# TaceoLabs/co-snarks

Measured on NVIDIA H100. Metric: co-Groth16 proofs/sec (BN254, 2^20 constraints); MSM Mscalar/s, higher is better.
Workload: dtype u32x8 (256-bit Montgomery, integer)

## Files before the change

co_snarks_b200/csrc/cs_msm.cuh:

```cuda
#pragma once
#include <stdlib.h>
#include "cs_common.cuh"
#include "cs_curve.cuh"

namespace cs {

constexpr unsigned MSM_SLICE_MAX = 64;
constexpr unsigned MSM_ORDER_BLOCK = 256;
constexpr unsigned MSM_RED_SEG = 4;
constexpr unsigned MSM_SIGN = 0x80000000u;

template <class FrP, class Fn>
CS_D void msm_recode(const uint32_t* __restrict__ scalars, uint32_t sstride, uint32_t i, int mont, uint32_t c,
                     uint32_t W, Fn&& f) {
  Fp<FrP> s;
  const uint4* src = reinterpret_cast<const uint4*>(scalars) + (size_t)i * sstride * (FrP::N / 4);
  CS_UNROLL
  for (int k = 0; k < FrP::N / 4; k++) {
    uint4 v = src[k];
    s.l[4 * k] = v.x; s.l[4 * k + 1] = v.y; s.l[4 * k + 2] = v.z; s.l[4 * k + 3] = v.w;
  }
  if (mont) s = s.from_mont();
  const uint32_t half = 1u << (c - 1);
  const uint32_t mask = (1u << c) - 1;
  uint32_t carry = 0;
  for (uint32_t w = 0; w < W; w++) {
    uint32_t pos = w * c;
    uint32_t li = pos >> 5, sh = pos & 31;
    uint32_t lo = li < FrP::N ? s.l[li] : 0;
    uint32_t hi = li + 1 < FrP::N ? s.l[li + 1] : 0;
    uint32_t d = (__funnelshift_r(lo, hi, sh) & mask) + carry;
    uint32_t out;
    if (d > half) {
      out = ((1u << c) - d) | MSM_SIGN;
      carry = 1;
    } else {
      out = d;
      carry = 0;
    }
    f(w, out);
  }
}

CS_D bool msm_base_inf(const uint32_t* __restrict__ infmask, uint32_t k) {
  return infmask && ((infmask[k >> 5] >> (k & 31)) & 1);
}

constexpr unsigned MSM_BIN_T = 1024;
constexpr unsigned MSM_BIN_TILE = 4096;
constexpr unsigned MSM_BIN_SPAN = 1u << 15;
constexpr unsigned MSM_SCATTER_SPAN = 1u << 13;

template <class FrP>
CS_GLOBAL void __launch_bounds__(MSM_BIN_T) k_msm_bin_count(const uint32_t* __restrict__ scalars, uint32_t sstride,
                                                            uint32_t n, int mont, uint32_t c, uint32_t W,
                                                            const uint32_t* __restrict__ infmask, uint32_t offset,
                                                            uint32_t tile, uint32_t B, uint32_t* __restrict__ tab) {
  CS_DYN_SMEM(uint32_t, h);
  const uint32_t lo = blockIdx.y * MSM_BIN_SPAN + 1;
  const uint32_t span = B + 1 - lo < MSM_BIN_SPAN ? B + 1 - lo : MSM_BIN_SPAN;
  for (uint32_t k = threadIdx.x; k < span; k += blockDim.x) h[k] = 0;
  __syncthreads();
  const uint32_t i1 = (blockIdx.x + 1) * tile < n ? (blockIdx.x + 1) * tile : n;
  for (uint32_t i = blockIdx.x * tile + threadIdx.x; i < i1; i += blockDim.x) {
    if (msm_base_inf(infmask, offset + i)) continue;
    msm_recode<FrP>(scalars, sstride, i, mont, c, W, [&](uint32_t, uint32_t d) {
      const uint32_t k = (d & ~MSM_SIGN) - lo;
      if (k < span) atomicAdd(&h[k], 1u);
    });
  }
  __syncthreads();
  uint32_t* row = tab + (size_t)blockIdx.x * B + (lo - 1);
  for (uint32_t k = threadIdx.x; k < span; k += blockDim.x) row[k] = h[k];
}

constexpr unsigned MSM_BIN_SCAN_U = 16;
static CS_GLOBAL void k_msm_bin_scan(uint32_t* __restrict__ tab, uint32_t nblk, uint32_t B, uint32_t* __restrict__ count) {
  const uint32_t b = blockIdx.x * blockDim.x + threadIdx.x;
  if (b == 0) count[0] = 0;
  if (b >= B) return;
  uint32_t* col = tab + b;
  uint32_t run = 0, r = 0;
  for (; r + MSM_BIN_SCAN_U <= nblk; r += MSM_BIN_SCAN_U) {
    uint32_t v[MSM_BIN_SCAN_U];
    CS_UNROLL
    for (uint32_t u = 0; u < MSM_BIN_SCAN_U; u++) v[u] = col[(size_t)(r + u) * B];
    CS_UNROLL
    for (uint32_t u = 0; u < MSM_BIN_SCAN_U; u++) {
      col[(size_t)(r + u) * B] = run;
      run += v[u];
    }
  }
  for (; r < nblk; r++) {
    const uint32_t v = col[(size_t)r * B];
    col[(size_t)r * B] = run;
    run += v;
  }
  count[b + 1] = run;
}

template <class FrP>
CS_GLOBAL void __launch_bounds__(MSM_BIN_T) k_msm_bin_scatter(const uint32_t* __restrict__ scalars, uint32_t sstride,
                                                              uint32_t n, int mont, uint32_t c, uint32_t W,
                                                              const uint32_t* __restrict__ infmask, uint32_t offset,
                                                              uint32_t tile, uint32_t B, uint32_t nbases,
                                                              const uint32_t* __restrict__ tab,
                                                              const uint32_t* __restrict__ start,
                                                              uint32_t* __restrict__ sorted) {
  CS_DYN_SMEM(uint32_t, cur);
  const uint32_t lo = blockIdx.y * MSM_SCATTER_SPAN + 1;
  const uint32_t span = B + 1 - lo < MSM_SCATTER_SPAN ? B + 1 - lo : MSM_SCATTER_SPAN;
  const uint32_t* row = tab + (size_t)blockIdx.x * B + (lo - 1);
  for (uint32_t k = threadIdx.x; k < span; k += blockDim.x) cur[k] = start[lo + k] + row[k];
  __syncthreads();
  const uint32_t i1 = (blockIdx.x + 1) * tile < n ? (blockIdx.x + 1) * tile : n;
  for (uint32_t i = blockIdx.x * tile + threadIdx.x; i < i1; i += blockDim.x) {
    if (msm_base_inf(infmask, offset + i)) continue;
    msm_recode<FrP>(scalars, sstride, i, mont, c, W, [&](uint32_t w, uint32_t d) {
      const uint32_t k = (d & ~MSM_SIGN) - lo;
      if (k < span) sorted[atomicAdd(&cur[k], 1u)] = (w * nbases + offset + i) | (d & MSM_SIGN);
    });
  }
}

template <class F>
CS_GLOBAL void k_msm_infmask(const Affine<F>* __restrict__ table, uint32_t n, uint32_t* __restrict__ mask) {
  uint32_t wd = blockIdx.x * blockDim.x + threadIdx.x;
  if (wd * 32 >= n) return;
  uint32_t m = 0;
  for (uint32_t k = 0; k < 32 && wd * 32 + k < n; k++)
    if (table[wd * 32 + k].is_inf()) m |= 1u << k;
  mask[wd] = m;
}

constexpr unsigned MSM_SCAN_T = 1024;
constexpr unsigned MSM_SCAN_MAX_BLOCKS = 1024;
CS_D void msm_scan_terms(const uint32_t* __restrict__ count, uint32_t k, uint32_t nb1, uint32_t S, uint32_t* v) {
  uint32_t cnt = (k && k < nb1) ? count[k] : 0;
  uint32_t n0 = (cnt + S - 1) / S;
  uint32_t n1 = (n0 + S - 1) / S;
  v[0] = cnt; v[1] = n0; v[2] = n1; v[3] = (n1 + S - 1) / S;
}
static CS_GLOBAL void k_msm_scan1(const uint32_t* __restrict__ count, uint32_t nb1 , uint32_t S,
                                  uint32_t* __restrict__ start, uint32_t* __restrict__ sstart0,
                                  uint32_t* __restrict__ sstart1, uint32_t* __restrict__ sstart2, uint32_t* __restrict__ aux) {
  __shared__ uint32_t sm[4][32];
  const uint32_t t = threadIdx.x, lane = t & 31, wid = t >> 5, nwarp = blockDim.x >> 5;
  const uint32_t k = blockIdx.x * blockDim.x + t;
  uint32_t v[4], inc[4];
  msm_scan_terms(count, k, nb1, S, v);
  CS_UNROLL
  for (int q = 0; q < 4; q++) {
    uint32_t x = v[q];
    CS_UNROLL
    for (uint32_t d = 1; d < 32; d <<= 1) {
      uint32_t y = __shfl_up_sync(0xffffffffu, x, d);
      if (lane >= d) x += y;
    }
    inc[q] = x;
    if (lane == 31) sm[q][wid] = x;
  }
  __syncthreads();
  uint32_t w[4], x[4];
  CS_UNROLL
  for (int q = 0; q < 4; q++) {
    w[q] = (wid == 0 && lane < nwarp) ? sm[q][lane] : 0;
    x[q] = w[q];
    CS_UNROLL
    for (uint32_t d = 1; d < 32; d <<= 1) {
      uint32_t y = __shfl_up_sync(0xffffffffu, x[q], d);
      if (lane >= d) x[q] += y;
    }
  }
  __syncthreads();
  if (wid == 0 && lane < nwarp) {
    CS_UNROLL
    for (int q = 0; q < 4; q++) sm[q][lane] = x[q] - w[q];
    if (lane == nwarp - 1) {
      CS_UNROLL
      for (int q = 0; q < 4; q++) aux[blockIdx.x * 4 + q] = x[q];
    }
  }
  __syncthreads();
  if (k < nb1) {
    start[k] = sm[0][wid] + inc[0] - v[0];
    sstart0[k] = sm[1][wid] + inc[1] - v[1];
    sstart1[k] = sm[2][wid] + inc[2] - v[2];
    sstart2[k] = sm[3][wid] + inc[3] - v[3];
  }
}
static CS_GLOBAL void k_msm_scan2(const uint32_t* __restrict__ count, uint32_t nb1, uint32_t S,
                                  uint32_t* __restrict__ start, uint32_t* __restrict__ sstart0,
                                  uint32_t* __restrict__ sstart1, uint32_t* __restrict__ sstart2,
                                  const uint32_t* __restrict__ aux) {
  const uint32_t k = blockIdx.x * blockDim.x + threadIdx.x;
  if (k >= nb1) return;
  uint32_t off[4] = {0, 0, 0, 0};
  for (uint32_t b = 0; b < blockIdx.x; b++) {
    CS_UNROLL
    for (int q = 0; q < 4; q++) off[q] += aux[b * 4 + q];
  }
  uint32_t a = start[k] + off[0], b0 = sstart0[k] + off[1], b1 = sstart1[k] + off[2], b2 = sstart2[k] + off[3];
  start[k] = a; sstart0[k] = b0; sstart1[k] = b1; sstart2[k] = b2;
  if (k == nb1 - 1) {
    uint32_t v[4];
    msm_scan_terms(count, k, nb1, S, v);
    start[nb1] = a + v[0]; sstart0[nb1] = b0 + v[1]; sstart1[nb1] = b1 + v[2]; sstart2[nb1] = b2 + v[3];
  }
}

constexpr unsigned MSM_VIEW_T = 256;
constexpr unsigned MSM_VIEW_WORDS = MSM_VIEW_T / 32;

CS_D uint32_t popc32(uint32_t x) {
#if defined(CS_EMU)
  return (uint32_t)__builtin_popcount(x);
#else
  return __popc(x);
#endif
}
CS_D uint32_t warp_bits(bool pred) {
#if defined(CS_EMU)
  uint32_t x = pred ? 1u << (threadIdx.x & 31) : 0u;
  for (uint32_t d = 16; d > 0; d >>= 1) x += __shfl_xor_sync(0xffffffffu, x, d);
  return x;
#else
  return __ballot_sync(0xffffffffu, pred);
#endif
}

static CS_GLOBAL void k_msm_view_flags(const uint32_t* __restrict__ sorted, const uint32_t* __restrict__ src_start,
                                       uint32_t nb1, uint32_t n, const uint32_t* __restrict__ infmask, uint32_t offset,
                                       uint32_t* __restrict__ keep, uint32_t* __restrict__ blk_cnt) {
  __shared__ uint32_t cnt[MSM_VIEW_WORDS];
  const uint32_t t = threadIdx.x;
  const uint32_t p = blockIdx.x * MSM_VIEW_T + t;
  bool k = false;
  if (p < src_start[nb1]) {
    const uint32_t i = (sorted[p] & ~MSM_SIGN) % n;
    k = !((infmask[(offset + i) >> 5] >> ((offset + i) & 31)) & 1);
  }
  const uint32_t bits = warp_bits(k);
  if ((t & 31) == 0) {
    keep[(size_t)blockIdx.x * MSM_VIEW_WORDS + (t >> 5)] = bits;
    cnt[t >> 5] = popc32(bits);
  }
  __syncthreads();
  if (t == 0) {
    uint32_t c = 0;
    for (uint32_t w = 0; w < MSM_VIEW_WORDS; w++) c += cnt[w];
    blk_cnt[blockIdx.x] = c;
  }
}

static CS_GLOBAL void k_msm_view_scan(const uint32_t* __restrict__ blk_cnt, uint32_t nblk, uint32_t* __restrict__ blk_off) {
  __shared__ uint32_t sm[MSM_SCAN_T];
  const uint32_t t = threadIdx.x, T = blockDim.x;
  const uint32_t per = (nblk + T - 1) / T;
  const uint32_t lo = t * per < nblk ? t * per : nblk, hi = lo + per < nblk ? lo + per : nblk;
  uint32_t s = 0;
  for (uint32_t b = lo; b < hi; b++) s += blk_cnt[b];
  sm[t] = s;
  __syncthreads();
  for (uint32_t d = 1; d < T; d <<= 1) {
    const uint32_t v = t >= d ? sm[t - d] : 0;
    __syncthreads();
    sm[t] += v;
    __syncthreads();
  }
  uint32_t run = sm[t] - s;
  for (uint32_t b = lo; b < hi; b++) {
    const uint32_t c = blk_cnt[b];
    blk_off[b] = run;
    run += c;
  }
  if (t == T - 1) blk_off[nblk] = run;
}

CS_D uint32_t view_kept_before(uint32_t p, const uint32_t* __restrict__ keep, const uint32_t* __restrict__ blk_off) {
  const uint32_t blk = p / MSM_VIEW_T;
  uint32_t r = blk_off[blk];
  for (uint32_t w = blk * MSM_VIEW_WORDS; w < (p >> 5); w++) r += popc32(keep[w]);
  if (p & 31) r += popc32(keep[p >> 5] & ((1u << (p & 31)) - 1));
  return r;
}

static CS_GLOBAL void k_msm_view_counts(const uint32_t* __restrict__ src_start, uint32_t nb1, const uint32_t* __restrict__ keep,
                                        const uint32_t* __restrict__ blk_off, uint32_t* __restrict__ count) {
  const uint32_t b = blockIdx.x * blockDim.x + threadIdx.x;
  if (b >= nb1) return;
  count[b] = b ? view_kept_before(src_start[b + 1], keep, blk_off) - view_kept_before(src_start[b], keep, blk_off) : 0;
}

static CS_GLOBAL void k_msm_view_scatter(const uint32_t* __restrict__ sorted, uint32_t n, uint32_t nbases, uint32_t offset,
                                         const uint32_t* __restrict__ keep, const uint32_t* __restrict__ blk_off,
                                         uint32_t* __restrict__ out) {
  const uint32_t t = threadIdx.x;
  const uint32_t* kb = keep + (size_t)blockIdx.x * MSM_VIEW_WORDS;
  const uint32_t word = kb[t >> 5];
  if (!((word >> (t & 31)) & 1)) return;
  uint32_t pos = blk_off[blockIdx.x] + popc32(word & ((1u << (t & 31)) - 1));
  for (uint32_t k = 0; k < (t >> 5); k++) pos += popc32(kb[k]);
  const uint32_t e = sorted[blockIdx.x * MSM_VIEW_T + t];
  const uint32_t v = e & ~MSM_SIGN, w = v / n, i = v - w * n;
  out[pos] = (w * nbases + offset + i) | (e & MSM_SIGN);
}

CS_D uint32_t find_bucket(const uint32_t* __restrict__ arr, uint32_t nb1, uint32_t s) {
  uint32_t lo = 0, hi = nb1;
  while (hi - lo > 1) {
    uint32_t mid = (lo + hi) >> 1;
    if (arr[mid] <= s) lo = mid; else hi = mid;
  }
  return lo;
}

static CS_GLOBAL void k_msm_slice_hist(const uint32_t* __restrict__ count, const uint32_t* __restrict__ sstart0,
                                       uint32_t nb1, uint32_t S, uint32_t* __restrict__ slice_len,
                                       uint32_t* __restrict__ slice_bkt, uint32_t* __restrict__ block_hist) {
  __shared__ uint32_t h[MSM_SLICE_MAX + 1];
  for (uint32_t k = threadIdx.x; k <= MSM_SLICE_MAX; k += blockDim.x) h[k] = 0;
  __syncthreads();
  uint32_t s = blockIdx.x * blockDim.x + threadIdx.x;
  if (s < sstart0[nb1]) {
    uint32_t lo = 0, hi = nb1;
    while (hi - lo > 1) {
      uint32_t mid = (lo + hi) >> 1;
      if (sstart0[mid] <= s) lo = mid; else hi = mid;
    }
    uint32_t j = s - sstart0[lo];
    uint32_t len = count[lo] - j * S;
    if (len > S) len = S;
    slice_len[s] = len;
    slice_bkt[s] = lo;
    atomicAdd(&h[len], 1u);
  }
  __syncthreads();
  for (uint32_t k = threadIdx.x; k <= MSM_SLICE_MAX; k += blockDim.x)
    block_hist[(size_t)blockIdx.x * (MSM_SLICE_MAX + 1) + k] = h[k];
}

constexpr unsigned MSM_OFF_CHUNKS = 64;
static CS_GLOBAL void k_msm_slice_off1(const uint32_t* __restrict__ block_hist, uint32_t nblocks,
                                       uint32_t* __restrict__ chunk_sum) {
  uint32_t id = blockIdx.x * blockDim.x + threadIdx.x;
  if (id >= (MSM_SLICE_MAX + 1) * MSM_OFF_CHUNKS) return;
  uint32_t L = id / MSM_OFF_CHUNKS, ch = id % MSM_OFF_CHUNKS;
  uint32_t per = (nblocks + MSM_OFF_CHUNKS - 1) / MSM_OFF_CHUNKS;
  uint32_t lo = ch * per, hi = lo + per < nblocks ? lo + per : nblocks;
  uint32_t sum = 0;
  for (uint32_t b = lo; b < hi; b++) sum += block_hist[(size_t)b * (MSM_SLICE_MAX + 1) + L];
  chunk_sum[id] = sum;
}
static CS_GLOBAL void k_msm_slice_off2(uint32_t* __restrict__ chunk_sum, uint32_t* __restrict__ len_base) {
  uint32_t L = blockIdx.x * blockDim.x + threadIdx.x;
  if (L > MSM_SLICE_MAX) return;
  uint32_t run = 0;
  for (uint32_t c = 0; c < MSM_OFF_CHUNKS; c++) {
    uint32_t v = chunk_sum[L * MSM_OFF_CHUNKS + c];
    chunk_sum[L * MSM_OFF_CHUNKS + c] = run;
    run += v;
  }
  len_base[MSM_SLICE_MAX + 1 + L] = run;
}
static CS_GLOBAL void k_msm_slice_off3(uint32_t* __restrict__ block_hist, uint32_t nblocks,
                                       const uint32_t* __restrict__ chunk_sum, uint32_t* __restrict__ len_base) {
  uint32_t id = blockIdx.x * blockDim.x + threadIdx.x;
  if (id == 0) {
    uint32_t run = 0;
    for (int k = MSM_SLICE_MAX; k >= 0; k--) { len_base[k] = run; run += len_base[MSM_SLICE_MAX + 1 + k]; }
  }
  if (id >= (MSM_SLICE_MAX + 1) * MSM_OFF_CHUNKS) return;
  uint32_t L = id / MSM_OFF_CHUNKS, ch = id % MSM_OFF_CHUNKS;
  uint32_t per = (nblocks + MSM_OFF_CHUNKS - 1) / MSM_OFF_CHUNKS;
  uint32_t lo = ch * per, hi = lo + per < nblocks ? lo + per : nblocks;
  uint32_t run = chunk_sum[id];
  for (uint32_t b = lo; b < hi; b++) {
    uint32_t v = block_hist[(size_t)b * (MSM_SLICE_MAX + 1) + L];
    block_hist[(size_t)b * (MSM_SLICE_MAX + 1) + L] = run;
    run += v;
  }
}

static CS_GLOBAL void k_msm_slice_order(const uint32_t* __restrict__ slice_len, const uint32_t* __restrict__ slice_bkt,
                                        uint32_t nslices_max, const uint32_t* __restrict__ sstart0, uint32_t nb1,
                                        const uint32_t* __restrict__ block_off, const uint32_t* __restrict__ len_base,
                                        uint32_t* __restrict__ order, uint32_t* __restrict__ order_b) {
  __shared__ uint32_t h[MSM_SLICE_MAX + 1];
  for (uint32_t k = threadIdx.x; k <= MSM_SLICE_MAX; k += blockDim.x) h[k] = 0;
  __syncthreads();
  uint32_t s = blockIdx.x * blockDim.x + threadIdx.x;
  if (s < sstart0[nb1]) {
    uint32_t len = slice_len[s];
    uint32_t rank = atomicAdd(&h[len], 1u);
    uint32_t pos = len_base[len] + block_off[(size_t)blockIdx.x * (MSM_SLICE_MAX + 1) + len] + rank;
    order[pos] = s;
    order_b[pos] = slice_bkt[s];
  }
}

template <class F, int MINB>
CS_GLOBAL void __launch_bounds__(128, MINB) k_msm_accum0(const Affine<F>* __restrict__ table,
                                                         const uint32_t* __restrict__ sorted,
                                                         const uint32_t* __restrict__ count,
                                                         const uint32_t* __restrict__ start,
                                                         const uint32_t* __restrict__ sstart0, uint32_t nb1, uint32_t S,
                                                         const uint32_t* __restrict__ order,
                                                         const uint32_t* __restrict__ order_b,
                                                         Xyzz<F>* __restrict__ part0) {
  uint32_t t = blockIdx.x * blockDim.x + threadIdx.x;
  if (t >= sstart0[nb1]) return;
  uint32_t s = order[t];
  uint32_t b = order_b[t];
  uint32_t j = s - sstart0[b];
  uint32_t beg = start[b] + j * S;
  uint32_t end = start[b] + count[b];
  if (end > beg + S) end = beg + S;
  Xyzz<F> acc = Xyzz<F>::inf();
  uint32_t e = sorted[beg];
  if constexpr (sizeof(Affine<F>) > 64) {
    for (uint32_t k = beg; k < end; k++) {
      const uint32_t e_cur = e;
      if (k + 1 < end) {
        e = sorted[k + 1];
        prefetch_l1(table + (e & ~MSM_SIGN));
      }
      madd(acc, table[e_cur & ~MSM_SIGN], (e_cur & MSM_SIGN) != 0);
    }
    part0[s] = acc;
    return;
  }
  Affine<F> p = table[e & ~MSM_SIGN];
  for (uint32_t k = beg; k < end; k++) {
    uint32_t e_cur = e;
    Affine<F> p_cur = p;
    if (k + 1 < end) {
      e = sorted[k + 1];
      p = table[e & ~MSM_SIGN];
    }
    madd(acc, p_cur, (e_cur & MSM_SIGN) != 0);
  }
  part0[s] = acc;
}

template <class F>
CS_GLOBAL void __launch_bounds__(128) k_msm_accum1(const Xyzz<F>* __restrict__ part0,
                                                   const uint32_t* __restrict__ sstart0,
                                                   const uint32_t* __restrict__ sstart1, uint32_t nb1, uint32_t S,
                                                   Xyzz<F>* __restrict__ part1) {
  uint32_t s = blockIdx.x * blockDim.x + threadIdx.x;
  if (s >= sstart1[nb1]) return;
  uint32_t b = find_bucket(sstart1, nb1, s);
  uint32_t j = s - sstart1[b];
  uint32_t beg = sstart0[b] + j * S;
  uint32_t end = sstart0[b + 1];
  if (end > beg + S) end = beg + S;
  Xyzz<F> acc = part0[beg];
  for (uint32_t k = beg + 1; k < end; k++) padd(acc, part0[k]);
  part1[s] = acc;
}

template <class F>
CS_GLOBAL void __launch_bounds__(128) k_msm_accum2(const Xyzz<F>* __restrict__ part1,
                                                   const uint32_t* __restrict__ sstart1, uint32_t nb1,
                                                   Xyzz<F>* __restrict__ bucket) {
  uint32_t b = blockIdx.x * blockDim.x + threadIdx.x;
  if (b >= nb1) return;
  uint32_t beg = sstart1[b], end = sstart1[b + 1];
  Xyzz<F> acc = Xyzz<F>::inf();
  if (beg < end) {
    acc = part1[beg];
    for (uint32_t k = beg + 1; k < end; k++) padd(acc, part1[k]);
  }
  bucket[b] = acc;
}

template <class F>
CS_GLOBAL void __launch_bounds__(128) k_msm_reduce_seg(const Xyzz<F>* __restrict__ bucket, uint32_t B,
                                                       uint32_t L, Xyzz<F>* __restrict__ red) {
  uint32_t t = blockIdx.x * blockDim.x + threadIdx.x;
  uint32_t lo = t * L;
  if (lo >= B) return;
  uint32_t hi = lo + L < B ? lo + L : B;
  Xyzz<F> acc = Xyzz<F>::inf(), tot = Xyzz<F>::inf();
  for (uint32_t b = hi; b > lo; b--) {
    padd(acc, bucket[b]);
    padd(tot, acc);
  }
  if (lo != 0 && !acc.is_inf()) {
    Xyzz<F> m = Xyzz<F>::inf();
    int top = 31 - __clz(lo);
    for (int bit = top; bit >= 0; bit--) {
      m = dbl_xyzz(m);
      if ((lo >> bit) & 1) padd(m, acc);
    }
    padd(tot, m);
  }
  red[t] = tot;
}

template <class F>
CS_GLOBAL void k_msm_final_sum(const Xyzz<F>* __restrict__ red, uint32_t cnt,
                                                      Xyzz<F>* __restrict__ out) {
  CS_DYN_SMEM(Xyzz<F>, sm);
  const uint32_t T = blockDim.x, t = threadIdx.x;
  Xyzz<F> acc = Xyzz<F>::inf();
  for (uint32_t k = blockIdx.x * T + t; k < cnt; k += gridDim.x * T) padd(acc, red[k]);
  sm[t] = acc;
  __syncthreads();
  for (uint32_t step = T >> 1; step > 0; step >>= 1) {
    if (t < step) {
      Xyzz<F> a = sm[t];
      padd(a, sm[t + step]);
      sm[t] = a;
    }
    __syncthreads();
  }
  if (t == 0) out[blockIdx.x] = sm[0];
}

constexpr int MSM_PRE_CHUNK = 8;
template <class F>
CS_GLOBAL void __launch_bounds__(128) k_msm_precompute(Affine<F>* __restrict__ table, uint32_t n,
                                                       uint32_t c, uint32_t W) {
  uint32_t i = blockIdx.x * blockDim.x + threadIdx.x;
  if (i >= n) return;
  Affine<F> p = table[i];
  if (p.is_inf()) {
    for (uint32_t w = 1; w < W; w++) table[(size_t)w * n + i] = Affine<F>::inf();
    return;
  }
  Xyzz<F> cur = Xyzz<F>::from_affine(p);
  uint32_t w = 1;
  while (w < W) {
    Xyzz<F> pts[MSM_PRE_CHUNK];
    F pre[MSM_PRE_CHUNK];
    int cnt = 0;
    bool degenerate = false;
    for (; cnt < MSM_PRE_CHUNK && w + cnt < W; cnt++) {
      for (uint32_t k = 0; k < c; k++) cur = dbl_xyzz(cur);
      pts[cnt] = cur;
      degenerate = degenerate || cur.is_inf();
    }
    Affine<F> last;
    if (degenerate) {
      for (int j = 0; j < cnt; j++) {
        last = to_affine(pts[j]);
        table[(size_t)(w + j) * n + i] = last;
      }
    } else {
      pre[0] = pts[0].zzz;
      for (int j = 1; j < cnt; j++) pre[j] = pre[j - 1] * pts[j].zzz;
      F inv = pre[cnt - 1].inverse();
      for (int j = cnt - 1; j >= 0; j--) {
        F zi = j ? inv * pre[j - 1] : inv;
        inv = inv * pts[j].zzz;
        F zzi = (zi * pts[j].zz).sqr();
        Affine<F> a;
        a.x = pts[j].x * zzi;
        a.y = pts[j].y * zi;
        table[(size_t)(w + j) * n + i] = a;
        if (j == cnt - 1) last = a;
      }
    }
    cur = Xyzz<F>::from_affine(last);
    w += cnt;
  }
}

template <class F, class FrP>
CS_GLOBAL void __launch_bounds__(128) k_fixed_base_mul(const Affine<F>* __restrict__ base,
                                                       const uint32_t* __restrict__ scalars, uint32_t n,
                                                       int mont, Affine<F>* __restrict__ out) {
  uint32_t i = blockIdx.x * blockDim.x + threadIdx.x;
  if (i >= n) return;
  Fp<FrP> s;
  const uint4* src = reinterpret_cast<const uint4*>(scalars) + (size_t)i * (FrP::N / 4);
  CS_UNROLL
  for (int k = 0; k < FrP::N / 4; k++) {
    uint4 v = src[k];
    s.l[4 * k] = v.x; s.l[4 * k + 1] = v.y; s.l[4 * k + 2] = v.z; s.l[4 * k + 3] = v.w;
  }
  if (mont) s = s.from_mont();
  uint32_t lim[FrP::N];
  CS_UNROLL
  for (int k = 0; k < FrP::N; k++) lim[k] = s.l[k];
  Affine<F> b = base[0];
  Xyzz<F> acc = Xyzz<F>::inf();
  for (int bit = FrP::N * 32 - 1; bit >= 0; bit--) {
    acc = dbl_xyzz(acc);
    if ((lim[bit >> 5] >> (bit & 31)) & 1) madd(acc, b, false);
  }
  out[i] = to_affine(acc);
}

struct MsmShape {
  uint32_t c, W, B;
};

static inline MsmShape msm_shape(uint32_t scalar_bits, uint32_t c) {
  MsmShape s;
  s.c = c;
  s.W = (scalar_bits + 1 + c - 1) / c;
  s.B = 1u << (c - 1);
  return s;
}

static inline uint32_t msm_auto_window(size_t n, uint32_t scalar_bits) {
  int lg = 0;
  while ((1ull << (lg + 1)) <= n) lg++;
  int c = lg >= 15 ? 16 : lg - 4;
  if (c < 4) c = 4;
  while (c < 16) {
    const uint32_t W = (scalar_bits + 1 + c - 1) / c;
    const uint32_t top = scalar_bits + 1 - (W - 1) * c;
    if (2 * top >= (uint32_t)c) break;
    c++;
  }
  return (uint32_t)c;
}
static inline uint32_t msm_slice(const MsmShape& sh) {
  const char* e = getenv("CS_MSM_SLICE");
  if (e && atoi(e) == 64) return 64u;
  if (e && atoi(e) == 32) return 32u;
  return sh.c >= 18 ? 64u : 32u;
}

constexpr int MSM_NSTAGE = 5;
struct MsmWorkspace {
  DevBuf dig, sorted, meta, part0, part1, part2, bucket, red, scal, result, order;
  void* h_result = nullptr;
  size_t h_result_cap = 0;
  bool profile = false;
  cudaEvent_t ev[MSM_NSTAGE + 1] = {};
  cudaEvent_t sorted_ev = nullptr;
  bool sorted_ev_made = false, sorted_once = false;
  cudaEvent_t acc_in = nullptr, acc_out = nullptr;
  int mark(int i, cudaStream_t st) {
    if (!profile) return 0;
    if (!ev[i]) CS_CUDA(cudaEventCreateWithFlags(&ev[i], 0));
    CS_CUDA(cudaEventRecord(ev[i], st));
    return 0;
  }
  void release() {
    for (int i = 0; i <= MSM_NSTAGE; i++) {
      if (ev[i]) cudaEventDestroy(ev[i]);
      ev[i] = nullptr;
    }
    if (sorted_ev_made) cudaEventDestroy(sorted_ev);
    if (acc_in) cudaEventDestroy(acc_in);
    if (acc_out) cudaEventDestroy(acc_out);
    acc_in = acc_out = nullptr;
    sorted_ev = nullptr;
    sorted_ev_made = sorted_once = false;
    dig.release(); sorted.release(); meta.release(); part0.release(); part1.release(); part2.release();
    bucket.release(); red.release(); scal.release(); result.release(); order.release();
    if (h_result) cudaFreeHost(h_result);
    h_result = nullptr;
    h_result_cap = 0;
  }
};

template <class F>
int msm_accum0_f52(const Affine<F>* table, const uint32_t* sorted, const uint32_t* count, const uint32_t* start,
                   const uint32_t* sstart0, uint32_t nb1, uint32_t S, const uint32_t* order, const uint32_t* order_b,
                   Xyzz<F>* part0, uint32_t max_s0, cudaStream_t st);

struct MsmSizes {
  uint32_t nb1, S, ob;
  size_t nent, max_s0, max_s1, max_s2;
  MsmSizes(const MsmShape& sh, uint32_t n) {
    nb1 = sh.B + 1;
    nent = (size_t)sh.W * n;
    S = msm_slice(sh);
    max_s0 = nent / S + nb1;
    max_s1 = max_s0 / S + nb1;
    max_s2 = max_s1 / S + nb1;
    ob = ceil_div(max_s0, MSM_ORDER_BLOCK);
  }
  size_t meta_words() const { return (size_t)nb1 + 4 * ((size_t)nb1 + 1) + 4 * MSM_SCAN_MAX_BLOCKS; }
  size_t order_words() const {
    return 4 * max_s0 + (size_t)ob * (MSM_SLICE_MAX + 1) + 2 * (MSM_SLICE_MAX + 1) + (size_t)(MSM_SLICE_MAX + 1) * MSM_OFF_CHUNKS;
  }
};
struct MsmSortBufs {
  uint32_t *count, *start, *sstart0, *sstart1, *sstart2, *aux;
  uint32_t *slice_len, *slice_bkt, *order, *order_b, *block_hist, *len_base, *chunk_sum;
  MsmSortBufs(const MsmWorkspace& w, const MsmSizes& z) {
    count = w.meta.as<uint32_t>();
    start = count + z.nb1;
    sstart0 = start + z.nb1 + 1;
    sstart1 = sstart0 + z.nb1 + 1;
    sstart2 = sstart1 + z.nb1 + 1;
    aux = sstart2 + z.nb1 + 1;
    slice_len = w.order.as<uint32_t>();
    slice_bkt = slice_len + z.max_s0;
    order = slice_bkt + z.max_s0;
    order_b = order + z.max_s0;
    block_hist = order_b + z.max_s0;
    len_base = block_hist + (size_t)z.ob * (MSM_SLICE_MAX + 1);
    chunk_sum = len_base + 2 * (MSM_SLICE_MAX + 1);
  }
};

static inline int msm_check_limits(const MsmShape& sh, uint32_t n, uint32_t nbases) {
  const size_t nent = (size_t)sh.W * n;
  if (nent >= (1ull << 31) || (size_t)sh.W * nbases >= (1ull << 31))
    return fail(-3, "msm: W*n = %zu exceeds 2^31 entries", nent);
  return 0;
}

static inline int msm_scan(const MsmSortBufs& q, const MsmSizes& z, uint32_t B, cudaStream_t st) {
  const uint32_t sb = ceil_div(z.nb1, MSM_SCAN_T);
  if (sb > MSM_SCAN_MAX_BLOCKS) return fail(-3, "msm: %u buckets exceed the scan's limit", B);
  CS_LAUNCH_SYNC(k_msm_scan1, sb, MSM_SCAN_T, 0, st, q.count, z.nb1, z.S, q.start, q.sstart0, q.sstart1, q.sstart2, q.aux);
  CS_LAUNCH(k_msm_scan2, sb, MSM_SCAN_T, 0, st, q.count, z.nb1, z.S, q.start, q.sstart0, q.sstart1, q.sstart2, q.aux);
  return 0;
}

static inline int msm_slice_order(MsmWorkspace& ws, const MsmSortBufs& q, const MsmSizes& z, cudaStream_t st) {
  CS_LAUNCH_SYNC(k_msm_slice_hist, z.ob, MSM_ORDER_BLOCK, 0, st, q.count, q.sstart0, z.nb1, z.S, q.slice_len, q.slice_bkt,
                 q.block_hist);
  const uint32_t nt = (MSM_SLICE_MAX + 1) * MSM_OFF_CHUNKS;
  CS_LAUNCH(k_msm_slice_off1, ceil_div(nt, 128), 128, 0, st, q.block_hist, z.ob, q.chunk_sum);
  CS_LAUNCH(k_msm_slice_off2, 1, 128, 0, st, q.chunk_sum, q.len_base);
  CS_LAUNCH(k_msm_slice_off3, ceil_div(nt, 128), 128, 0, st, q.block_hist, z.ob, q.chunk_sum, q.len_base);
  CS_LAUNCH_SYNC(k_msm_slice_order, z.ob, MSM_ORDER_BLOCK, 0, st, q.slice_len, q.slice_bkt, (uint32_t)z.max_s0, q.sstart0,
                 z.nb1, q.block_hist, q.len_base, q.order, q.order_b);
  if (!ws.sorted_ev_made) {
    CS_CUDA(cudaEventCreateWithFlags(&ws.sorted_ev, cudaEventDisableTiming));
    ws.sorted_ev_made = true;
  }
  CS_CUDA(cudaEventRecord(ws.sorted_ev, st));
  ws.sorted_once = true;
  return 0;
}

template <class FrP>
int msm_smem_optin() {
#if !defined(CS_EMU)
  CS_CUDA(cudaFuncSetAttribute(k_msm_bin_count<FrP>, cudaFuncAttributeMaxDynamicSharedMemorySize, MSM_BIN_SPAN * 4));
  CS_CUDA(cudaFuncSetAttribute(k_msm_bin_scatter<FrP>, cudaFuncAttributeMaxDynamicSharedMemorySize, MSM_SCATTER_SPAN * 4));
#endif
  return 0;
}

static inline uint32_t msm_bin_tile(const MsmShape& sh, const MsmSizes& z, uint32_t n) {
  const size_t rows = z.nent / sh.B > 1 ? z.nent / sh.B : 1;
  const size_t nblk = ceil_div(n, MSM_BIN_TILE) < rows ? ceil_div(n, MSM_BIN_TILE) : rows;
  return n ? ceil_div(n, nblk) : 1;
}

template <class FrP>
int msm_sort(MsmWorkspace& ws, const uint32_t* infmask, uint32_t nbases, MsmShape sh, uint32_t offset,
             const uint32_t* d_scalars, uint32_t sstride, uint32_t n, int mont, cudaStream_t st) {
  CS_TRY(msm_check_limits(sh, n, nbases));
  const MsmSizes z(sh, n);
  const uint32_t tile = msm_bin_tile(sh, z, n);
  const uint32_t nblk = n ? ceil_div(n, tile) : 0;
  const dim3 grid(nblk, ceil_div(sh.B, MSM_BIN_SPAN)), grid_sc(nblk, ceil_div(sh.B, MSM_SCATTER_SPAN));
  const uint32_t smem = (sh.B < MSM_BIN_SPAN ? sh.B : MSM_BIN_SPAN) * 4;
  const uint32_t smem_sc = (sh.B < MSM_SCATTER_SPAN ? sh.B : MSM_SCATTER_SPAN) * 4;
  const size_t tab_words = (size_t)nblk * sh.B;
  CS_TRY(ws.dig.reserve((tab_words > z.nent ? tab_words : z.nent) * 4));
  CS_TRY(ws.sorted.reserve(z.nent * 4));
  CS_TRY(ws.meta.reserve(z.meta_words() * 4));
  CS_TRY(ws.order.reserve(z.order_words() * 4));
  const MsmSortBufs q(ws, z);
  uint32_t* tab = ws.dig.as<uint32_t>();
  CS_TRY(ws.mark(0, st));
  if (nblk)
    CS_LAUNCH_SYNC(k_msm_bin_count<FrP>, grid, MSM_BIN_T, smem, st, d_scalars, sstride, n, mont, sh.c, sh.W, infmask,
                   offset, tile, sh.B, tab);
  CS_TRY(ws.mark(1, st));
  CS_LAUNCH(k_msm_bin_scan, ceil_div(sh.B, 256), 256, 0, st, tab, nblk, sh.B, q.count);
  CS_TRY(msm_scan(q, z, sh.B, st));
  if (nblk)
    CS_LAUNCH_SYNC(k_msm_bin_scatter<FrP>, grid_sc, MSM_BIN_T, smem_sc, st, d_scalars, sstride, n, mont, sh.c, sh.W, infmask,
                   offset, tile, sh.B, nbases, tab, q.start, ws.sorted.as<uint32_t>());
  return msm_slice_order(ws, q, z, st);
}

static inline int msm_view(MsmWorkspace& ws, const MsmWorkspace& src, const uint32_t* infmask, uint32_t nbases,
                           MsmShape sh, uint32_t offset, uint32_t n, cudaStream_t st) {
  const MsmSizes z(sh, n);
  const uint32_t nblk = ceil_div(z.nent, MSM_VIEW_T);
  CS_TRY(ws.dig.reserve(((size_t)nblk * MSM_VIEW_WORDS + 2 * (size_t)nblk + 1) * 4));
  CS_TRY(ws.sorted.reserve(z.nent * 4));
  CS_TRY(ws.meta.reserve(z.meta_words() * 4));
  CS_TRY(ws.order.reserve(z.order_words() * 4));
  const MsmSortBufs q(ws, z), s(src, z);
  uint32_t* keep = ws.dig.as<uint32_t>();
  uint32_t* blk_cnt = keep + (size_t)nblk * MSM_VIEW_WORDS;
  uint32_t* blk_off = blk_cnt + nblk;
  const uint32_t* src_sorted = src.sorted.as<uint32_t>();
  CS_LAUNCH_SYNC(k_msm_view_flags, nblk, MSM_VIEW_T, 0, st, src_sorted, s.start, z.nb1, n, infmask, offset, keep, blk_cnt);
  CS_LAUNCH_SYNC(k_msm_view_scan, 1, MSM_SCAN_T, 0, st, blk_cnt, nblk, blk_off);
  CS_LAUNCH(k_msm_view_counts, ceil_div(z.nb1, 256), 256, 0, st, s.start, z.nb1, keep, blk_off, q.count);
  CS_LAUNCH(k_msm_view_scatter, nblk, MSM_VIEW_T, 0, st, src_sorted, n, nbases, offset, keep, blk_off,
            ws.sorted.as<uint32_t>());
  CS_TRY(msm_scan(q, z, sh.B, st));
  return msm_slice_order(ws, q, z, st);
}

template <class F, class FrP>
int msm_enqueue(MsmWorkspace& ws, const Affine<F>* table, const uint32_t* infmask, uint32_t nbases, MsmShape sh,
                uint32_t offset,
                const uint32_t* d_scalars, uint32_t sstride, uint32_t n, int mont, cudaStream_t st,
                MsmWorkspace* sort_from = nullptr, bool view = false, bool table_m260 = false, cudaStream_t st_acc = nullptr) {
  CS_TRY(msm_check_limits(sh, n, nbases));
  const MsmSizes z(sh, n);
  const uint32_t nb1 = z.nb1, S = z.S;
  const size_t max_s0 = z.max_s0, max_s1 = z.max_s1, max_s2 = z.max_s2;
  CS_TRY(ws.part0.reserve(max_s0 * sizeof(Xyzz<F>)));
  CS_TRY(ws.part1.reserve(max_s1 * sizeof(Xyzz<F>)));
  CS_TRY(ws.part2.reserve(max_s2 * sizeof(Xyzz<F>)));
  CS_TRY(ws.bucket.reserve((size_t)nb1 * sizeof(Xyzz<F>)));
  const uint32_t L = sh.B < MSM_RED_SEG ? sh.B : MSM_RED_SEG;
  const uint32_t nseg = (sh.B + L - 1) / L;
  const uint32_t fs_threads = sizeof(Xyzz<F>) > 128 ? 128 : 256;
  const uint32_t fs_blocks = nseg > 4 * fs_threads ? (nseg + fs_threads - 1) / fs_threads : 1;
  CS_TRY(ws.red.reserve(((size_t)nseg + fs_blocks) * sizeof(Xyzz<F>)));
  CS_TRY(ws.result.reserve(sizeof(Xyzz<F>)));
  if (ws.h_result_cap < sizeof(Xyzz<F>)) {
    if (ws.h_result) cudaFreeHost(ws.h_result);
    CS_CUDA(cudaMallocHost(&ws.h_result, sizeof(Xyzz<F>)));
    ws.h_result_cap = sizeof(Xyzz<F>);
  }
  if (sort_from) {
    if (!sort_from->sorted_once) return fail(-1, "msm: the workspace to share a sort with has not been enqueued");
    CS_TRY(ws.mark(0, st));
    CS_CUDA(cudaStreamWaitEvent(st, sort_from->sorted_ev, 0));
    CS_TRY(ws.mark(1, st));
    if (view) CS_TRY(msm_view(ws, *sort_from, infmask, nbases, sh, offset, n, st));
  } else {
    CS_TRY(msm_sort<FrP>(ws, infmask, nbases, sh, offset, d_scalars, sstride, n, mont, st));
  }
  MsmWorkspace& so = sort_from && !view ? *sort_from : ws;
  const MsmSortBufs q(so, z);
  const uint32_t *count = q.count, *start = q.start, *sstart0 = q.sstart0, *sstart1 = q.sstart1, *sstart2 = q.sstart2;
  const uint32_t *order = q.order, *order_b = q.order_b;
  CS_TRY(ws.mark(2, st));
  cudaStream_t st_main = st;
  if (st_acc) {
    if (!ws.acc_in) {
      CS_CUDA(cudaEventCreateWithFlags(&ws.acc_in, cudaEventDisableTiming));
      CS_CUDA(cudaEventCreateWithFlags(&ws.acc_out, cudaEventDisableTiming));
    }
    CS_CUDA(cudaEventRecord(ws.acc_in, st));
    CS_CUDA(cudaStreamWaitEvent(st_acc, ws.acc_in, 0));
    st = st_acc;
  }
  {
    static int minb_env = -1;
    if (minb_env < 0) { const char* e = getenv("CS_ACCUM0_MINB"); minb_env = e ? atoi(e) : 0; }
    const int minb = minb_env ? minb_env : (sizeof(Affine<F>) > 64 ? 2 : 4);
    if (table_m260) {
      CS_TRY((msm_accum0_f52<F>(table, so.sorted.as<uint32_t>(), count, start, sstart0, nb1, S, order, order_b,
                                ws.part0.as<Xyzz<F>>(), (uint32_t)max_s0, st)));
    } else {
#define CS_ACC0(M)                                                                                              \
  CS_LAUNCH(k_msm_accum0<F COMMA M>, ceil_div(max_s0, 128), 128, 0, st, table, so.sorted.as<uint32_t>(), count, \
            start, sstart0, nb1, S, order, order_b, ws.part0.as<Xyzz<F>>())
    switch (minb) {
      case 2: CS_ACC0(2); break;
      case 3: CS_ACC0(3); break;
      case 5: CS_ACC0(5); break;
      case 6: CS_ACC0(6); break;
      default: CS_ACC0(4); break;
    }
#undef CS_ACC0
    }
  }
  if (st_acc) {
    CS_CUDA(cudaEventRecord(ws.acc_out, st_acc));
    st = st_main;
    CS_CUDA(cudaStreamWaitEvent(st, ws.acc_out, 0));
  }
  CS_TRY(ws.mark(3, st));
  CS_LAUNCH(k_msm_accum1<F>, ceil_div(max_s1, 128), 128, 0, st, ws.part0.as<Xyzz<F>>(), sstart0, sstart1,
            nb1, S, ws.part1.as<Xyzz<F>>());
  CS_LAUNCH(k_msm_accum1<F>, ceil_div(max_s2, 128), 128, 0, st, ws.part1.as<Xyzz<F>>(), sstart1, sstart2,
            nb1, S, ws.part2.as<Xyzz<F>>());
  CS_LAUNCH(k_msm_accum2<F>, ceil_div(nb1, 128), 128, 0, st, ws.part2.as<Xyzz<F>>(), sstart2, nb1,
            ws.bucket.as<Xyzz<F>>());
  CS_TRY(ws.mark(4, st));
  CS_LAUNCH(k_msm_reduce_seg<F>, ceil_div(nseg, 128), 128, 0, st, ws.bucket.as<Xyzz<F>>(), sh.B, L,
            ws.red.as<Xyzz<F>>());
  if (fs_blocks > 1) {
    Xyzz<F>* stage = ws.red.as<Xyzz<F>>() + nseg;
    CS_LAUNCH_SYNC(k_msm_final_sum<F>, fs_blocks, fs_threads, fs_threads * sizeof(Xyzz<F>), st, ws.red.as<Xyzz<F>>(), nseg,
                   stage);
    CS_LAUNCH_SYNC(k_msm_final_sum<F>, 1, fs_threads, fs_threads * sizeof(Xyzz<F>), st, stage, fs_blocks,
                   ws.result.as<Xyzz<F>>());
  } else {
    CS_LAUNCH_SYNC(k_msm_final_sum<F>, 1, fs_threads, fs_threads * sizeof(Xyzz<F>), st, ws.red.as<Xyzz<F>>(), nseg,
                   ws.result.as<Xyzz<F>>());
  }
  CS_TRY(ws.mark(5, st));
  CS_CUDA(cudaMemcpyAsync(ws.h_result, ws.result.p, sizeof(Xyzz<F>), cudaMemcpyDeviceToHost, st));
  CS_CUDA(cudaGetLastError());
  return 0;
}

}
```

Baseline: 51.41.

## Replace segmented bucket reduction with tree-based weighted sum kernel

Replaces the per-thread segment reduction (which ran a double-and-add loop to multiply each segment's sum by its offset) and the separate final-sum kernel with a single multi-level tree kernel. Each tree node carries a pair (weighted sum, plain sum times span), combined with point additions and a doubling, so the weighted bucket sum comes out of a log-depth reduction. This removes the serial scalar-multiplication tail per segment and the sequential per-thread bucket loops. In exchange it adds more passes through shared memory with synchronisation, extra launches for large bucket counts, and several additions per node.

```diff
diff --git a/co_snarks_b200/csrc/cs_msm.cuh b/co_snarks_b200/csrc/cs_msm.cuh
--- a/co_snarks_b200/csrc/cs_msm.cuh
+++ b/co_snarks_b200/csrc/cs_msm.cuh
@@ -7,7 +7,6 @@
 
 constexpr unsigned MSM_SLICE_MAX = 64;
 constexpr unsigned MSM_ORDER_BLOCK = 256;
-constexpr unsigned MSM_RED_SEG = 4;
 constexpr unsigned MSM_SIGN = 0x80000000u;
 
 template <class FrP, class Fn>
@@ -476,47 +475,48 @@
 }
 
 template <class F>
-CS_GLOBAL void __launch_bounds__(128) k_msm_reduce_seg(const Xyzz<F>* __restrict__ bucket, uint32_t B,
-                                                       uint32_t L, Xyzz<F>* __restrict__ red) {
-  uint32_t t = blockIdx.x * blockDim.x + threadIdx.x;
-  uint32_t lo = t * L;
-  if (lo >= B) return;
-  uint32_t hi = lo + L < B ? lo + L : B;
-  Xyzz<F> acc = Xyzz<F>::inf(), tot = Xyzz<F>::inf();
-  for (uint32_t b = hi; b > lo; b--) {
-    padd(acc, bucket[b]);
-    padd(tot, acc);
-  }
-  if (lo != 0 && !acc.is_inf()) {
-    Xyzz<F> m = Xyzz<F>::inf();
-    int top = 31 - __clz(lo);
-    for (int bit = top; bit >= 0; bit--) {
-      m = dbl_xyzz(m);
-      if ((lo >> bit) & 1) padd(m, acc);
-    }
-    padd(tot, m);
-  }
-  red[t] = tot;
-}
-
-template <class F>
-CS_GLOBAL void k_msm_final_sum(const Xyzz<F>* __restrict__ red, uint32_t cnt,
-                                                      Xyzz<F>* __restrict__ out) {
+CS_GLOBAL void k_msm_weigh(const Xyzz<F>* __restrict__ bucket, const Xyzz<F>* __restrict__ in, uint32_t nleaf,
+                           Xyzz<F>* __restrict__ out) {
   CS_DYN_SMEM(Xyzz<F>, sm);
-  const uint32_t T = blockDim.x, t = threadIdx.x;
-  Xyzz<F> acc = Xyzz<F>::inf();
-  for (uint32_t k = blockIdx.x * T + t; k < cnt; k += gridDim.x * T) padd(acc, red[k]);
-  sm[t] = acc;
-  __syncthreads();
-  for (uint32_t step = T >> 1; step > 0; step >>= 1) {
-    if (t < step) {
-      Xyzz<F> a = sm[t];
-      padd(a, sm[t + step]);
-      sm[t] = a;
-    }
+  const uint32_t T = blockDim.x, i = threadIdx.x;
+  Xyzz<F>* sq = sm;
+  Xyzz<F>* sp = sm + T;
+  const uint32_t k = 2 * (blockIdx.x * T + i);
+  auto leaf = [&](uint32_t j, int which) -> Xyzz<F> {
+    if (j >= nleaf) return Xyzz<F>::inf();
+    return bucket ? bucket[j + 1] : in[2 * j + which];
+  };
+  Xyzz<F> x = leaf(k, 0);
+  padd(x, leaf(k + 1, 0));
+  padd(x, leaf(k + 1, 1));
+  sq[i] = x;
+  x = leaf(k, 1);
+  padd(x, leaf(k + 1, 1));
+  sp[i] = dbl_xyzz(x);
+  const uint32_t h = T >> 1;
+  for (uint32_t step = 1; step < T; step <<= 1) {
     __syncthreads();
-  }
-  if (t == 0) out[blockIdx.x] = sm[0];
+    const uint32_t nodes = T / (2 * step);
+    const uint32_t r = i < h ? i : i - h;
+    if (r < nodes) {
+      const uint32_t l = r * 2 * step;
+      if (i < h) {
+        Xyzz<F> q = sq[l];
+        padd(q, sq[l + step]);
+        padd(q, sp[l + step]);
+        sq[l] = q;
+      } else if (nodes > 1 || gridDim.x > 1) {
+        Xyzz<F> p = sp[l];
+        padd(p, sp[l + step]);
+        sp[l] = dbl_xyzz(p);
+      }
+    }
+  }
+  __syncthreads();
+  if (i == 0) {
+    out[2 * blockIdx.x] = sq[0];
+    out[2 * blockIdx.x + 1] = sp[0];
+  }
 }
 
 constexpr int MSM_PRE_CHUNK = 8;
@@ -816,12 +816,10 @@
   CS_TRY(ws.part1.reserve(max_s1 * sizeof(Xyzz<F>)));
   CS_TRY(ws.part2.reserve(max_s2 * sizeof(Xyzz<F>)));
   CS_TRY(ws.bucket.reserve((size_t)nb1 * sizeof(Xyzz<F>)));
-  const uint32_t L = sh.B < MSM_RED_SEG ? sh.B : MSM_RED_SEG;
-  const uint32_t nseg = (sh.B + L - 1) / L;
-  const uint32_t fs_threads = sizeof(Xyzz<F>) > 128 ? 128 : 256;
-  const uint32_t fs_blocks = nseg > 4 * fs_threads ? (nseg + fs_threads - 1) / fs_threads : 1;
-  CS_TRY(ws.red.reserve(((size_t)nseg + fs_blocks) * sizeof(Xyzz<F>)));
-  CS_TRY(ws.result.reserve(sizeof(Xyzz<F>)));
+  const uint32_t wt = sizeof(Xyzz<F>) > 128 ? 64 : 128;
+  const uint32_t wblk = ceil_div(sh.B, 2 * wt);
+  CS_TRY(ws.red.reserve(2 * ((size_t)wblk + ceil_div(wblk, 2 * wt)) * sizeof(Xyzz<F>)));
+  CS_TRY(ws.result.reserve(2 * sizeof(Xyzz<F>)));
   if (ws.h_result_cap < sizeof(Xyzz<F>)) {
     if (ws.h_result) cudaFreeHost(ws.h_result);
     CS_CUDA(cudaMallocHost(&ws.h_result, sizeof(Xyzz<F>)));
@@ -885,17 +883,20 @@
   CS_LAUNCH(k_msm_accum2<F>, ceil_div(nb1, 128), 128, 0, st, ws.part2.as<Xyzz<F>>(), sstart2, nb1,
             ws.bucket.as<Xyzz<F>>());
   CS_TRY(ws.mark(4, st));
-  CS_LAUNCH(k_msm_reduce_seg<F>, ceil_div(nseg, 128), 128, 0, st, ws.bucket.as<Xyzz<F>>(), sh.B, L,
-            ws.red.as<Xyzz<F>>());
-  if (fs_blocks > 1) {
-    Xyzz<F>* stage = ws.red.as<Xyzz<F>>() + nseg;
-    CS_LAUNCH_SYNC(k_msm_final_sum<F>, fs_blocks, fs_threads, fs_threads * sizeof(Xyzz<F>), st, ws.red.as<Xyzz<F>>(), nseg,
-                   stage);
-    CS_LAUNCH_SYNC(k_msm_final_sum<F>, 1, fs_threads, fs_threads * sizeof(Xyzz<F>), st, stage, fs_blocks,
-                   ws.result.as<Xyzz<F>>());
-  } else {
-    CS_LAUNCH_SYNC(k_msm_final_sum<F>, 1, fs_threads, fs_threads * sizeof(Xyzz<F>), st, ws.red.as<Xyzz<F>>(), nseg,
-                   ws.result.as<Xyzz<F>>());
+  {
+    Xyzz<F>* nodes[2] = {ws.red.as<Xyzz<F>>(), ws.red.as<Xyzz<F>>() + 2 * (size_t)wblk};
+    const Xyzz<F>* bucket = ws.bucket.as<Xyzz<F>>();
+    const Xyzz<F>* in = nullptr;
+    uint32_t nleaf = sh.B;
+    for (int k = 0;; k++) {
+      const uint32_t nblk = ceil_div(nleaf, 2 * wt);
+      Xyzz<F>* out = nblk == 1 ? ws.result.as<Xyzz<F>>() : nodes[k & 1];
+      CS_LAUNCH_SYNC(k_msm_weigh<F>, nblk, wt, 2 * wt * sizeof(Xyzz<F>), st, bucket, in, nleaf, out);
+      if (nblk == 1) break;
+      bucket = nullptr;
+      in = out;
+      nleaf = nblk;
+    }
   }
   CS_TRY(ws.mark(5, st));
   CS_CUDA(cudaMemcpyAsync(ws.h_result, ws.result.p, sizeof(Xyzz<F>), cudaMemcpyDeviceToHost, st));
```

New measurement: 51.72, median of 6. Within noise of the previous version (+0.6%).
